# FDzhaozi/HiD-VAE

Measured on AMD Instinct MI355X. Metric: item-embeddings/sec HiD-VAE train step, 768-d in, 3x256 codebooks, higher is better.
Workload: dtype f32; 1 GPU; Amazon-Beauty-shaped synthetic 768-d, 3x256 codebooks, batch 1024/GPU, ROTATION_TRICK, tagged (projector+InfoNCE+predictor+focal/mixup: the step both h-configs run) train step = fwd+bwd+AdamW(cosine); global_batch=1024, parallelism=dp1, hip_graph=True, graph_queues=3, GPU_MAX_HW_QUEUES=4, collectives_in_graph=False

## Files before the change

hid-vae_amd/_C.py:

```python
import ctypes
import os

import torch

_HERE = os.path.dirname(os.path.abspath(__file__))
LIB_PATH = os.path.join(_HERE, "libhidvae_hip.so")
_lib = None

MODE_GUMBEL, MODE_STE, MODE_ROTATION = 1, 2, 3
DIST_L2, DIST_COSINE = 0, 1
GEMM_NT, GEMM_NN, GEMM_TN = 0, 1, 2
EPI_NONE, EPI_SILU, EPI_RELU, EPI_GELU, EPI_SIGMOID = 0, 1, 2, 3, 4
EPI_DSILU, EPI_DRELU, EPI_DGELU, EPI_DSIGMOID = 16, 17, 18, 19
MAX_LEVELS = 8
EMBED_DIM = 32

_vp, _i, _i64, _f, _u32 = ctypes.c_void_p, ctypes.c_int, ctypes.c_int64, ctypes.c_float, ctypes.c_uint32

_SIGNATURES = {
    "hidvae_gemm_f32": [_i, _i64, _i64, _i64, _vp, _i64, _vp, _i64, _vp, _vp, _i64, _i, _vp, _i64, _vp, _i64, _f, _vp, _u32, _u32, _i, _vp, _i, _vp],
    "hidvae_linear_bwd": [_vp, _i64, _vp, _i64, _vp, _i64, _i64, _i64, _i64, _vp, _i64, _i, _vp, _i64, _i, _vp, _i64, _f, _vp, _i, _vp, _i, _vp],
    "hidvae_layernorm_bwd_partial": [_vp, _vp, _vp, _vp, _vp, _vp, _i64, _i64, _i, _vp, _f, _f, _vp, _vp, _vp, _vp, _vp],
    "hidvae_layernorm_param_final_many": [_vp, _i, _vp],
    "hidvae_predictor_fwd": [_vp, _i64, _i64, _vp, _i, _vp, _vp],
    "hidvae_predictor_bwd": [_vp, _i64, _i64, _vp, _i, _vp, _i64, _vp],
    "hidvae_gate_fwd": [_vp, _i64, _i64, _i, _vp, _vp, _vp, _vp, _vp, _vp, _i, _f, _vp, _vp, _vp, _vp, _vp, _vp, _vp],
    "hidvae_gate_bwd": [_vp, _i64, _vp, _i64, _i64, _i, _vp, _vp, _vp, _i, _f, _vp, _vp, _vp, _vp, _vp, _vp, _vp, _vp, _vp],
    "hidvae_colsum": [_vp, _i64, _i64, _i64, _vp, _i, _vp, _vp],
    "hidvae_codebook_prepare": [_vp, _vp, _i, _i64, _vp, _vp, _i, _vp],
    "hidvae_rq_forward": [_vp, _i64, _i, _vp, _vp, _i, _i64, _i, _i, _f, _vp, _vp, _vp, _i64, _vp, _vp, _vp, _vp, _i, _i, _vp],
    "hidvae_bottleneck_fwd": [_vp, _i64, _i, _i, _vp, _vp, _vp, _vp, _vp, _i, _vp, _vp, _i, _i64, _i, _f, _vp, _vp, _vp, _i64, _vp, _vp,
                              _i, _i, _vp, _vp, _vp, _vp, _vp, _vp, _vp, _vp, _vp, _vp],
    "hidvae_rq_backward": [_vp, _vp, _i64, _i, _vp, _vp, _i, _i64, _i, _f, _vp, _vp, _i64, _vp, _vp, _i64, _f, _vp, _i64, _vp, _vp, _i, _vp],
    "hidvae_rq_backward_slices": [_vp, _vp, _i64, _i, _vp, _vp, _i, _i64, _i, _f, _vp, _vp, _vp, _i, _vp, _vp, _i64, _f, _vp, _i64, _vp, _vp, _i, _vp],
    "hidvae_uniq_loss": [_vp, _vp, _i64, _i, _f, _f, _vp, _vp, _i, _vp],
    "hidvae_total_loss": [_vp, _vp, _i64, _vp, _vp, _vp, _i, _f, _vp, _vp, _i, _f, _f, _f, _f, _f, _vp, _vp, _vp, _vp, _vp, _i, _vp],
    "hidvae_total_loss_bwd": [_vp, _i64, _i, _f, _f, _f, _vp, _vp, _vp, _i, _vp],
    "hidvae_codebook_grad": [_vp, _vp, _i64, _i, _i64, _vp, _vp, _vp, _vp, _i, _vp, _i, _vp],
    "hidvae_l2norm_fwd_pair": [_vp, _i64, _i64, _vp, _vp, _vp, _i64, _i64, _vp, _vp, _i64, _f, _vp],
    "hidvae_l2norm_bwd_pair": [_vp, _i64, _vp, _vp, _i64, _vp, _vp, _i64, _vp, _vp, _i64, _vp, _i64, _f, _vp],
    "hidvae_recon_fwd_bwd": [_vp, _vp, _i64, _i64, _i, _f, _vp, _i64, _vp, _vp, _vp, _vp],
    "hidvae_l2norm_fwd": [_vp, _i64, _i64, _i64, _f, _vp, _i64, _vp, _vp],
    "hidvae_l2norm32_fwd": [_vp, _i64, _i64, _f, _vp, _i64, _vp, _vp],
    "hidvae_l2norm_bwd": [_vp, _i64, _vp, _i64, _vp, _i64, _i64, _f, _vp, _i64, _i, _vp],
    "hidvae_id_stats": [_vp, _i64, _vp, _i64, _i, _vp, _vp, _vp, _i, _vp],
    "hidvae_act_bwd": [_vp, _vp, _i64, _i, _vp, _f, _vp, _vp],
    "hidvae_binary": [_i, _vp, _i64, _vp, _i64, _i64, _i64, _vp, _i64, _vp],
    "hidvae_sum_prefix_slices": [_vp, _vp, _i, _i64, _i64, _vp, _vp],
    "hidvae_layernorm_fwd": [_vp, _i64, _i64, _vp, _vp, _f, _vp, _vp, _vp, _i, _vp, _f, _vp, _vp, _u32, _u32, _vp],
    "hidvae_rng_advance": [_vp, _vp],
    "hidvae_dropout_mask": [_vp, _i64, _vp, _u32, _u32, _vp],
    "hidvae_layernorm_bwd": [_vp, _vp, _vp, _vp, _vp, _vp, _i64, _i64, _i, _vp, _f, _vp, _vp],
    "hidvae_layernorm_param_grad": [_vp, _vp, _vp, _vp, _vp, _vp, _i64, _i64, _i, _vp, _f, _vp, _vp, _i, _vp, _vp],
    "hidvae_layernorm_bwd_all": [_vp, _vp, _vp, _vp, _vp, _vp, _i64, _i64, _i, _vp, _f, _vp, _vp, _vp, _i, _vp, _vp],
    "hidvae_batchnorm_fwd": [_vp, _i64, _i64, _i64, _vp, _vp, _f, _f, _i, _vp, _vp, _vp, _vp, _vp, _vp, _i, _vp, _f, _vp, _u32, _u32, _vp, _vp],
    "hidvae_batchnorm_bwd": [_vp, _vp, _i64, _vp, _vp, _vp, _vp, _i64, _i64, _i, _vp, _f, _vp, _vp, _vp, _vp, _i, _vp, _vp],
    "hidvae_infonce_rows": [_vp, _i64, _f, _f, _vp, _vp, _vp],
    "hidvae_infonce_dlogits": [_vp, _i64, _f, _f, _vp, _vp],
    "hidvae_infonce_lse_chunk": [_vp, _i64, _i64, _i64, _i64, _f, _vp, _vp, _vp, _i, _vp],
    "hidvae_infonce_lse_finish": [_vp, _vp, _vp, _i64, _f, _f, _vp, _vp, _vp, _vp],
    "hidvae_infonce_dlogits_chunk": [_vp, _i64, _i64, _i64, _i64, _f, _f, _vp, _vp, _vp],
    "hidvae_mixup_plan": [_vp, _i64, _i, _i64, _vp, _f, _vp, _vp, _vp, _vp, _vp],
    "hidvae_tag_loss_fwd": [_vp, _i64, _i64, _vp, _vp, _vp, _i, _f, _f, _f, _f, _vp, _vp, _vp, _vp, _vp, _vp, _vp, _vp, _vp],
    "hidvae_tag_loss_bwd": [_vp, _vp, _vp, _vp, _vp, _i64, _i64, _vp, _vp, _vp, _vp],
    "hidvae_kmeans_iter": [_vp, _i64, _vp, _i64, _vp, _vp, _vp, _vp, _vp, _i, _vp],
    "hidvae_gumbel_rows_fwd": [_vp, _vp, _vp, _vp, _i64, _i64, _f, _vp, _i, _i, _vp],
    "hidvae_gumbel_loss": [_vp, _vp, _i64, _f, _vp, _i, _vp],
    "hidvae_gumbel_gemb": [_vp, _vp, _i64, _vp, _vp, _i64, _vp, _i, _vp],
    "hidvae_gumbel_rows_bwd": [_vp, _vp, _i64, _i64, _f, _vp, _vp],
    "hidvae_gumbel_finish": [_vp, _vp, _vp, _vp, _vp, _i64, _f, _i64, _vp, _vp, _vp, _i64, _i, _vp],
    "hidvae_cat_recon_rows": [_vp, _i64, _vp, _i64, _i64, _i64, _i, _vp, _i64, _vp, _vp, _vp],
    "hidvae_loss_fwd": [_vp, _vp, _i64, _i64, _i, _vp, _vp, _vp, _vp, _i, _f, _vp, _vp, _i, _f, _f, _f, _f, _f, _vp, _vp, _vp, _vp, _vp, _vp, _i, _vp],
    "hidvae_loss_bwd": [_vp, _vp, _vp, _i64, _i64, _i, _i, _f, _f, _f, _vp, _vp, _vp, _vp, _i, _f, _vp],
    "hidvae_padded_to_jagged": [_vp, _i64, _i64, _vp, _vp, _i64, _i64, _i64, _vp],
    "hidvae_jagged_to_padded": [_vp, _vp, _vp, _i64, _i64, _i64, _i64, _i64, _vp],
    "hidvae_gather_rows": [_vp, _i64, _i, _vp, _vp, _vp, _vp, _vp],
    "hidvae_codebook_prepare_adamw": [_vp, _vp, _i, _i64, _vp, _vp, _vp, _vp, _vp, _i, _f, _f, _f, _i64, _i64, _f, _vp, _i, _vp],
    "hidvae_adamw_prepare": [_vp, _vp, _vp, _i, _f, _f, _f, _i64, _i64, _f, _vp, _vp],
    "hidvae_adamw_step": [_vp, _vp, _vp, _vp, _vp, _vp, _i, _i64, _f, _f, _f, _f, _vp],
    "hidvae_query_workspace": [_i, _vp, _i, _vp],
    "hidvae_sqdiff_rows": [_vp, _i64, _vp, _i64, _i64, _i64, _f, _vp, _vp],
    "hidvae_sqdiff_rows_bwd": [_vp, _i64, _vp, _i64, _vp, _i64, _i64, _i64, _f, _f, _vp, _vp, _vp],
    "hidvae_gumbel_noise": [_vp, _i64, _f, _vp, _vp],
    "hidvae_gumbel_softmax_rows": [_vp, _vp, _i64, _i64, _f, _vp, _vp],
    "hidvae_softmax_argmax_rows": [_vp, _i64, _i64, _i64, _vp, _i64, _vp, _i64, _vp],
    "hidvae_timestamp": [_vp, _vp],
    "hidvae_linear_bwd_group": [_vp, _i, _vp],
    "hidvae_gemm_bf16": [_i64, _i64, _i64, _vp, _i64, _vp, _i64, _vp, _vp, _i64, _i, _vp, _i64, _vp, _i64, _f, _vp, _u32, _u32, _vp, _i, _vp],
    "hidvae_linear_bwd_bf16": [_vp, _i64, _vp, _i64, _vp, _i64, _i64, _i64, _i64, _vp, _i64, _i, _vp, _i64, _i, _vp, _i64, _f, _vp, _i, _vp, _vp],
    "hidvae_linear_bwd_group_bf16": [_vp, _i, _vp],
}
WS_GEMM, WS_LINEAR_BWD, WS_COLSUM, WS_CODEBOOK_GRAD, WS_LAYERNORM_PARAM_GRAD, WS_LAYERNORM_BWD_ALL = 1, 2, 3, 4, 5, 6
WS_BATCHNORM_FWD, WS_BATCHNORM_BWD, WS_ID_CENSUS, WS_KMEANS, WS_TAG_LOSS, WS_LINEAR_BWD_ZEROED, WS_RQ_FORWARD = 7, 8, 9, 10, 11, 12, 13
WS_LINEAR_BWD_BF16, WS_GEMM_BF16, WS_BF16_ZEROED = 14, 15, 16
PRECISIONS = ("fp32", "bf16")


class LaunchStamps:
    TICK_US = 0.01

    def __init__(self, device, capacity=4096):
        self.buf = torch.zeros((2 * capacity,), dtype=torch.int64, device=device)
        self.names, self.dims = [], []
        self.streams = []

    def _slot(self, name, dims=None, stream=None):
        if 2 * len(self.names) + 2 > self.buf.numel():
            raise RuntimeError("LaunchStamps: capacity exceeded")
        self.names.append(name)
        self.dims.append(dims)
        self.streams.append(int(getattr(stream, "value", stream) or 0))
        return self.buf.data_ptr() + 16 * (len(self.names) - 1)

    def rows(self):
        t = self.buf[: 2 * len(self.names)].cpu().reshape(-1, 2)
        d = ((t[:, 1] - t[:, 0]).double() * self.TICK_US).tolist()
        empty = [v for n, v in zip(self.names, d) if n == "(empty)"]
        base = sorted(empty)[len(empty) // 2] if empty else 0.0
        return [(n, v - base) for n, v in zip(self.names, d) if n != "(empty)"], base

    def spans(self):
        t = self.buf[: 2 * len(self.names)].cpu().reshape(-1, 2).double() * self.TICK_US
        t0 = float(t[:, 0].min()) if len(self.names) else 0.0
        return [(n, s, float(a) - t0, float(b) - t0) for n, s, (a, b) in zip(self.names, self.streams, t.tolist()) if n != "(empty)"]

    def rows_with_dims(self):
        rows, base = self.rows()
        dims = [dm for n, dm in zip(self.names, self.dims) if n != "(empty)"]
        return [(n, v, dm) for (n, v), dm in zip(rows, dims)], base


class PhaseMarks:

    def __init__(self, device, capacity=512):
        self.buf = torch.zeros((capacity,), dtype=torch.int64, device=device)
        self.labels = []

    def rows(self):
        t = self.buf[: len(self.labels)].cpu().double() * LaunchStamps.TICK_US
        t0 = float(t.min()) if len(self.labels) else 0.0
        return [(lab, st, float(v) - t0) for (lab, st), v in zip(self.labels, t.tolist())]


_PHASES = None


def phases_begin(device, capacity=512):
    global _PHASES
    _PHASES = PhaseMarks(device, capacity)
    return _PHASES


def phases_end():
    global _PHASES
    p, _PHASES = _PHASES, None
    return p


def phase_mark(label):
    p = _PHASES
    if p is None:
        return
    i = len(p.labels)
    if i >= p.buf.numel():
        raise RuntimeError("PhaseMarks: capacity exceeded")
    st = torch.cuda.current_stream().cuda_stream
    p.labels.append((label, int(st)))
    lib()._L.hidvae_timestamp(ctypes.c_void_p(p.buf.data_ptr() + 8 * i), ctypes.c_void_p(st))


_STAMPS = None
_NOT_LAUNCHES = ("hidvae_last_error", "hidvae_version", "hidvae_query_workspace", "hidvae_timestamp")


def stamps_begin(device, capacity=4096):
    global _STAMPS
    _STAMPS = LaunchStamps(device, capacity)
    return _STAMPS


def stamps_end():
    global _STAMPS
    st, _STAMPS = _STAMPS, None
    return st


def stamp_empty_bracket():
    st = _STAMPS
    if st is not None:
        p = st._slot("(empty)")
        lib()._L.hidvae_timestamp(ctypes.c_void_p(p), _stream())
        lib()._L.hidvae_timestamp(ctypes.c_void_p(p + 8), _stream())


def _gemm_dims(name, a):
    if name == "hidvae_gemm_f32":
        return (int(a[1]), int(a[2]), int(a[3]), 2.0 * a[1] * a[2] * a[3])
    if name == "hidvae_gemm_bf16":
        return (int(a[0]), int(a[1]), int(a[2]), 2.0 * a[0] * a[1] * a[2])
    if name in ("hidvae_linear_bwd", "hidvae_linear_bwd_bf16"):
        B, n_out, n_in = int(a[6]), int(a[7]), int(a[8])
        return (B, n_out, n_in, (4.0 if a[12] is not None else 2.0) * B * n_out * n_in)
    if name == "hidvae_bottleneck_fwd":
        B, K2, N2, L, K, Nd0, Nd1 = int(a[1]), int(a[2]), int(a[3]), int(a[12]), int(a[13]), int(a[22]), int(a[23])
        D = EMBED_DIM
        return (B, N2, K2, 2.0 * B * (K2 * N2 + N2 * D + L * K * D + D * Nd0 + Nd0 * Nd1))
    return None


class _LibProxy:

    def __init__(self, L):
        self._L = L

    def __getattr__(self, name):
        fn = getattr(self._L, name)
        if name in _NOT_LAUNCHES or not name.startswith("hidvae_"):
            return fn
        L = self._L

        def call(*a):
            st = _STAMPS
            if st is None:
                return fn(*a)
            p = st._slot(name, _gemm_dims(name, a), a[-1])
            L.hidvae_timestamp(ctypes.c_void_p(p), a[-1])
            rc = fn(*a)
            L.hidvae_timestamp(ctypes.c_void_p(p + 8), a[-1])
            return rc

        setattr(self, name, call)
        return call


def lib():
    global _lib
    if _lib is None:
        if not os.path.exists(LIB_PATH):
            raise RuntimeError(
                f"HIP extension missing: {LIB_PATH}. Build it with `python -c 'import __graft_entry__ as g; g.build()'` "
                "(hipcc --offload-arch=gfx950). There is no CPU fallback on the product path.")
        L = ctypes.CDLL(LIB_PATH)
        L.hidvae_last_error.restype = ctypes.c_char_p
        L.hidvae_version.restype = ctypes.c_char_p
        for name, sig in _SIGNATURES.items():
            fn = getattr(L, name)
            fn.argtypes = sig
            fn.restype = ctypes.c_int
        _lib = _LibProxy(L)
    return _lib


def exported_symbols():
    return ["hidvae_version", "hidvae_last_error"] + list(_SIGNATURES)

# ... 1056 lines not shown
```

hid-vae_amd/csrc/gemm.hip:

```cpp
#include <stdlib.h>
#include <type_traits>
#include "common.h"
#include "rules.h"
#include "gemm_ring.h"

namespace {

constexpr int BK = 16;

struct GemmArgs {
    int64_t M, N, K;
    const float *A;
    int64_t lda;
    const float *B;
    int64_t ldb;
    const float *bias;
    float *C;
    int64_t ldc;
    int epilogue;
    float *aux;
    int64_t ldaux;
    int accumulate;
    int64_t k_per_split;
    float *partial;
// ... 1262 lines not shown
        for (int v = 0; v < NV; v++) {
            f32x4 x = pf[slot][v];
            const int k = s * T16_BKS + k4[v];
            if (k + 4 > Ki) {
#pragma unroll
                for (int e = 0; e < 4; e++) x[e] = k + e < Ki ? x[e] : 0.0f;
            }
            *reinterpret_cast<f32x4 *>(base + dst[v]) = x;
        }
    };
    f32x4 acc = {0.f, 0.f, 0.f, 0.f};
    f32x4 fa[2][4], fb[2][4];
    auto frags = [&](int fs, int buf) {
        const float *As = lds + buf * BUF + (16 * wm + i16) * T16_STR + 4 * q;
        const float *Bs = lds + buf * BUF + A_SZ + (16 * wn + i16) * T16_STR + 4 * q;
#pragma unroll
        for (int u = 0; u < 4; u++) {
            fa[fs][u] = *reinterpret_cast<const f32x4 *>(As + 16 * u);
            fb[fs][u] = *reinterpret_cast<const f32x4 *>(Bs + 16 * u);
        }
    };
#pragma unroll
    for (int p = 0; p < PF; p++) fetch(p, p);
    stash(0, 0, 0);
    fetch(0, PF);
    stash(1 % PF, 1, 1);
    fetch(1 % PF, PF + 1);
    __syncthreads();
    frags(0, 0);
    constexpr int UN = 6;
    for (int s0 = 0; s0 < nsteps; s0 += UN) {
#pragma unroll
        for (int u = 0; u < UN; u++) {
            const int s = s0 + u;
            if (s < nsteps) {
                const int nblk = (Ki - s * T16_BKS + 15) / 16;
#pragma unroll
                for (int s4 = 0; s4 < 4; s4++) acc = __builtin_amdgcn_mfma_f32_16x16x4f32(fa[u & 1][0][s4], fb[u & 1][0][s4], acc, 0, 0, 0);
                __builtin_amdgcn_sched_barrier(0);
                if (s + 1 < nsteps) frags((u + 1) & 1, (u + 1) % NB);
                __builtin_amdgcn_sched_barrier(0);
#pragma unroll
                for (int b = 1; b < 4; b++)
                    if (b < nblk) {
#pragma unroll
                        for (int s4 = 0; s4 < 4; s4++) acc = __builtin_amdgcn_mfma_f32_16x16x4f32(fa[u & 1][b][s4], fb[u & 1][b][s4], acc, 0, 0, 0);
                    }
                if (s + 2 < nsteps) {
                    stash((u + 2) % PF, s + 2, (u + 2) % NB);
                    fetch((u + 2) % PF, s + 2 + PF);
                }
                __syncthreads();
            }
        }
    }
    const int64_t col = n0 + 16 * wn + i16;
    if (col >= g.N) return;
    const float bias = g.bias != nullptr ? g.bias[col] : 0.0f;
    const float *mk = g.mask;
#pragma unroll
    for (int r = 0; r < 4; r++) {
        const int64_t row = m0 + 16 * wm + 4 * q + r;
        if (row >= g.M) continue;
        float v = acc[r] + bias;
        if (g.aux != nullptr && g.epilogue < HIDVAE_EPI_DSILU && g.epilogue != HIDVAE_EPI_NONE) g.aux[row * g.ldaux + col] = v;
        v = apply_epilogue(g.epilogue, v, g.aux, row * g.ldaux + col, g.mask_scale);
        if (has_dropout(g)) v = v * dropout_factor(g, row, col);
        float *dstp = g.C + row * g.ldc + col;
        *dstp = g.accumulate ? *dstp + v : v;
    }
}

template <int WM, int WN>
int launch_tile16(const GemmArgs &g, hipStream_t s) {
    constexpr size_t bytes = (size_t)3 * (16 * WM + 16 * WN) * T16_STR * 4;
    static const hipError_t attr = hipFuncSetAttribute(reinterpret_cast<const void *>(&gemm_tile16_kernel<WM, WN>),
                                                       hipFuncAttributeMaxDynamicSharedMemorySize, (int)bytes);
    if (attr != hipSuccess) return -1;
    const int64_t tiles = hv_cdiv(g.M, 16 * WM) * hv_cdiv(g.N, 16 * WN);
    hipLaunchKernelGGL((gemm_tile16_kernel<WM, WN>), dim3((unsigned)tiles), dim3(64 * WM * WN), bytes, s, g);
    return 0;
}

template <int SPLIT>
void launch_directL(int layout, const GemmArgs &g, hipStream_t s) {
    dim3 grid((unsigned)hv_cdiv(g.N, 32), (unsigned)hv_cdiv(g.M, 32));
    dim3 block(64 * SPLIT);
    if (layout == HIDVAE_GEMM_NT) hipLaunchKernelGGL((gemm_directL_kernel<HIDVAE_GEMM_NT, SPLIT>), grid, block, 0, s, g);
    else hipLaunchKernelGGL((gemm_directL_kernel<HIDVAE_GEMM_NN, SPLIT>), grid, block, 0, s, g);
}

template <int SPLIT, int NS, int NWN = 1>
void launch_direct(int layout, const GemmArgs &g, hipStream_t s) {
    dim3 grid((unsigned)hv_cdiv(hv_cdiv(g.N, 32), NWN), (unsigned)hv_cdiv(g.M, 32));
    dim3 block(64 * SPLIT * NWN);
    if (layout == HIDVAE_GEMM_NT) hipLaunchKernelGGL((gemm_direct_kernel<HIDVAE_GEMM_NT, SPLIT, NS, NWN>), grid, block, 0, s, g);
    else if (layout == HIDVAE_GEMM_NN) hipLaunchKernelGGL((gemm_direct_kernel<HIDVAE_GEMM_NN, SPLIT, NS, NWN>), grid, block, 0, s, g);
    else hipLaunchKernelGGL((gemm_direct_kernel<HIDVAE_GEMM_TN, SPLIT, NS, NWN>), grid, block, 0, s, g);
}

template <int WM, int WN>
void launch_tile(int layout, const GemmArgs &g, int splits, hipStream_t s) {
    dim3 grid((unsigned)hv_cdiv(g.N, 32 * WN), (unsigned)hv_cdiv(g.M, 32 * WM), (unsigned)splits);
    dim3 block(64 * WM * WN);
    if (layout == HIDVAE_GEMM_NT) hipLaunchKernelGGL((gemm_f32_kernel<WM, WN, HIDVAE_GEMM_NT>), grid, block, 0, s, g);
    else if (layout == HIDVAE_GEMM_NN) hipLaunchKernelGGL((gemm_f32_kernel<WM, WN, HIDVAE_GEMM_NN>), grid, block, 0, s, g);
    else hipLaunchKernelGGL((gemm_f32_kernel<WM, WN, HIDVAE_GEMM_TN>), grid, block, 0, s, g);
}

inline bool aligned16(const void *p) { return (reinterpret_cast<uintptr_t>(p) & 15) == 0; }

inline bool fits32bit(int layout, int64_t M, int64_t N, int64_t K, int64_t lda, int64_t ldb) {
    const int64_t a_rows = (layout == HIDVAE_GEMM_TN) ? K : M, b_rows = (layout == HIDVAE_GEMM_NT) ? N : K;
    return a_rows * lda < (1ll << 29) && b_rows * ldb < (1ll << 29);
}
inline bool use_direct16(int64_t M, int64_t N, int64_t K) {
    const int64_t tiles32 = hv_cdiv(M, 32) * hv_cdiv(N, 32);
    return tiles32 <= 256 || (tiles32 <= 512 && K <= 256);
}
inline int pick_split32(int64_t M, int64_t N, int64_t K, int split_k) {
    const int64_t tiles32 = hv_cdiv(M, 32) * hv_cdiv(N, 32);
    int sp = 1;
    if (split_k != 1) {
        const int cap = split_k == 0 ? 16 : split_k;
        while (sp < cap && sp < 16 && tiles32 * sp < 2048 && K / (sp * 2) >= 32) sp *= 2;
    }
    return sp;
}
inline int pick_split16(int64_t M, int64_t N, int64_t K, int split_k) {
    const int64_t tiles16 = hv_cdiv(M, 16) * hv_cdiv(N, 16);
    int sp16 = 1;
    if (split_k != 1) {
        const int cap = split_k == 0 ? 16 : split_k;
        while (sp16 < cap && sp16 < 16 && tiles16 * sp16 < 4096 && K / (sp16 * 2) >= 32) sp16 *= 2;
    }
    return sp16;
}

constexpr int GROUP_MAX = 12;
constexpr int GROUP_WAVES = 8;
struct GroupSub {
    GemmArgs g;
    int kind;
    int layout, split, deep, nbx;
    int64_t nt;
    int nb;
};
struct GroupArgs {
    int n;
    GroupSub s[GROUP_MAX];
};

__device__ __forceinline__ void colsum_group_body(const GemmArgs &g, int64_t c0, float *part) {
    const int col = threadIdx.x & 31, rg = threadIdx.x >> 5, nrg = (int)(blockDim.x >> 5);
    const int64_t c = c0 + col;
    float acc = 0.0f;
    if (c < g.N)
        for (int64_t r0 = rg; r0 < g.M; r0 += 8 * (int64_t)nrg) {
            float v[8];
#pragma unroll
            for (int j = 0; j < 8; j++) v[j] = r0 + (int64_t)nrg * j < g.M ? g.A[(r0 + (int64_t)nrg * j) * g.lda + c] : 0.0f;
#pragma unroll
            for (int j = 0; j < 8; j++) acc += v[j];
        }
    part[rg * 32 + col] = acc;
    __syncthreads();
    if (threadIdx.x < 32 && c < g.N) {
        float v = part[col];
        for (int j = 1; j < nrg; j++) v += part[j * 32 + col];
        g.C[c] = g.accumulate ? g.C[c] + v : v;
    }
}

__global__ __launch_bounds__(64 * GROUP_WAVES) void gemm_group_kernel(GroupArgs a) {
    __shared__ float part[GROUP_WAVES * 1024];
    int bid = blockIdx.x, p = 0;
    while (p + 1 < a.n && bid >= a.s[p].nb) {
        bid -= a.s[p].nb;
        p++;
    }
    const GroupSub &s = a.s[p];
    if (s.kind == 2) {
        colsum_group_body(s.g, (int64_t)bid * 32, part);
        return;
    }
    const int64_t tile0 = (int64_t)xcd_slot(bid, s.nb) * (GROUP_WAVES / s.split);
    if (s.kind == 0) {
        if (s.layout == HIDVAE_GEMM_NT) {
            if (s.deep) direct16_body<HIDVAE_GEMM_NT, 6>(s.g, s.split, tile0, s.nt, s.nbx, part);
            else direct16_body<HIDVAE_GEMM_NT, 3>(s.g, s.split, tile0, s.nt, s.nbx, part);
        } else if (s.layout == HIDVAE_GEMM_NN) direct16_body<HIDVAE_GEMM_NN, 3>(s.g, s.split, tile0, s.nt, s.nbx, part);
        else direct16_body<HIDVAE_GEMM_TN, 3>(s.g, s.split, tile0, s.nt, s.nbx, part);
    } else {
        if (s.layout == HIDVAE_GEMM_NT) {
            if (s.deep) direct32_body<HIDVAE_GEMM_NT, 6>(s.g, s.split, tile0, s.nt, s.nbx, part);
            else direct32_body<HIDVAE_GEMM_NT, 3>(s.g, s.split, tile0, s.nt, s.nbx, part);
        } else if (s.layout == HIDVAE_GEMM_NN) {
            if (s.deep) direct32_body<HIDVAE_GEMM_NN, 6>(s.g, s.split, tile0, s.nt, s.nbx, part);
            else direct32_body<HIDVAE_GEMM_NN, 3>(s.g, s.split, tile0, s.nt, s.nbx, part);
        } else direct32_body<HIDVAE_GEMM_TN, 3>(s.g, s.split, tile0, s.nt, s.nbx, part);
    }
}

inline bool group_gemm_sub(GroupSub &s, int layout, const GemmArgs &g) {
    if (!fits32bit(layout, g.M, g.N, g.K, g.lda, g.ldb) || hv_cdiv(g.M, 32) * hv_cdiv(g.N, 32) >= 2048) return false;
    s.g = g;
    s.layout = layout;
    const bool f16 = use_direct16(g.M, g.N, g.K);
    s.kind = f16 ? 0 : 1;
    int sp = f16 ? pick_split16(g.M, g.N, g.K, 0) : pick_split32(g.M, g.N, g.K, 0);
    const int cap = hv_cdiv(g.M, 16) * hv_cdiv(g.N, 16) <= 16 ? GROUP_WAVES : 4;
    if (sp > GROUP_WAVES) sp = GROUP_WAVES;
    while (sp > cap && sp > 1) sp /= 2;
    s.split = sp;
    s.deep = g.K / (16 * sp) >= 12;
    const int T = f16 ? 16 : 32;
    s.nbx = (int)hv_cdiv(g.N, T);
    s.nt = (int64_t)s.nbx * hv_cdiv(g.M, T);
    s.nb = (int)hv_cdiv(s.nt, GROUP_WAVES / sp);
    return true;
}

inline int launch_group(GroupArgs &a, hipStream_t s) {
    int64_t blocks = 0;
    for (int i = 0; i < a.n; i++) blocks += a.s[i].nb;
    if (blocks == 0) return HIDVAE_OK;
    hipLaunchKernelGGL(gemm_group_kernel, dim3((unsigned)blocks), dim3(64 * GROUP_WAVES), 0, s, a);
    HV_LAUNCH_CHECK("gemm_group");
    return HIDVAE_OK;
}

}

extern "C" int hidvae_gemm_f32(int layout, int64_t M, int64_t N, int64_t K, const float *A, int64_t lda,
                               const float *B, int64_t ldb, const float *bias, float *C, int64_t ldc, int epilogue,
                               float *aux, int64_t ldaux, const float *mask, int64_t ldmask, float mask_scale,
                               const unsigned long long *rng_state, unsigned rng_site, unsigned drop_threshold,
                               int split_k, float *workspace, int accumulate, void *stream) {
    HV_REQUIRE(layout >= 0 && layout <= 2, "gemm: layout %d", layout);
    HV_REQUIRE(!(mask && rng_state), "gemm: a keep-mask OR the in-kernel generator, not both");
    HV_REQUIRE(M >= 1 && N >= 1 && K >= 1, "gemm: empty problem M=%lld N=%lld K=%lld", (long long)M, (long long)N, (long long)K);
    HV_REQUIRE(A && B && C, "gemm: null operand");
    const int64_t a_min = (layout == HIDVAE_GEMM_TN) ? M : K, b_min = (layout == HIDVAE_GEMM_NT) ? K : N;
    HV_REQUIRE(lda >= a_min && ldb >= b_min && ldc >= N, "gemm: leading dimension too small (lda=%lld ldb=%lld ldc=%lld)",
               (long long)lda, (long long)ldb, (long long)ldc);
    HV_REQUIRE(epilogue < HIDVAE_EPI_DSILU || (aux != nullptr && ldaux >= N), "gemm: backward epilogue %d needs aux", epilogue);
    HV_REQUIRE(mask == nullptr || ldmask >= N, "gemm: ldmask=%lld", (long long)ldmask);
    HV_REQUIRE(split_k >= 0, "gemm: split_k=%d", split_k);
    GemmArgs g{};
    g.M = M; g.N = N; g.K = K; g.A = A; g.lda = lda; g.B = B; g.ldb = ldb; g.bias = bias; g.C = C; g.ldc = ldc;
    g.epilogue = epilogue; g.aux = aux; g.ldaux = aux ? ldaux : 0; g.accumulate = accumulate;
    g.vecA = (lda % 4 == 0) && aligned16(A);
    g.vecB = (ldb % 4 == 0) && aligned16(B);
    g.mask = mask; g.ldmask = ldmask; g.mask_scale = mask_scale;
    g.drop = HvDrop{rng_state, rng_site, drop_threshold};
    hipStream_t s = (hipStream_t)stream;
    const int64_t tiles32 = hv_cdiv(M, 32) * hv_cdiv(N, 32);
    const bool fits32 = fits32bit(layout, M, N, K, lda, ldb);
    int deep_splits = 0;
    if (split_k == 0 && workspace != nullptr && K >= 4096 && tiles32 < 2048 && M > 32 && N > 32) {
        deep_splits = (int)(K / 512 < 16 ? K / 512 : 16);
        const int64_t wgs = hv_cdiv(M, 64) * hv_cdiv(N, 64);
        while (deep_splits > 2 && wgs * deep_splits > 2048) deep_splits /= 2;
    }
    const bool big = (tiles32 >= 2048 && K >= 64) || !fits32 || deep_splits > 1;
    if (!big || split_k == 1) {
        if (!big) {
            const int64_t nt16 = hv_cdiv(M, 16) * hv_cdiv(N, 16);
            const int64_t t_small = hv_cdiv(M, 32) * hv_cdiv(N, 64), t_big = hv_cdiv(M, 64) * hv_cdiv(N, 64);
            const bool fit_small = t_small >= 192 && t_small <= 256, fit_big = t_big >= 224 && t_big <= 256;
            if (layout == HIDVAE_GEMM_NT && split_k == 0 && K >= 256 && tiles32 >= 448) {
                HV_REQUIRE((launch_tile16<4, 4>(g, s)) == 0, "gemm_f32: could not size the LDS of gemm_tile16_kernel");
                HV_LAUNCH_CHECK("gemm_f32 tile16");
                return HIDVAE_OK;
            }
            if (layout == HIDVAE_GEMM_NT && split_k == 1 && K >= 256 && (fit_small || fit_big)) {
                const int rc = !fit_small ? launch_tile16<4, 4>(g, s) : launch_tile16<2, 4>(g, s);
                HV_REQUIRE(rc == 0, "gemm_f32: could not size the LDS of gemm_tile16_kernel");
                HV_LAUNCH_CHECK("gemm_f32 tile16");
                return HIDVAE_OK;
            }
            if (layout == HIDVAE_GEMM_NT && nt16 >= 512 && nt16 <= 8192 && K >= 64 && (split_k == 1 || (use_direct16(M, N, K) && K >= 128))) {
                constexpr int W16 = 4;
                hipLaunchKernelGGL(gemm_directL16_kernel<W16>, dim3((unsigned)hv_cdiv(nt16, W16)), dim3(64 * W16), 0, s, g);
                HV_LAUNCH_CHECK("gemm_f32 directL16");
                return HIDVAE_OK;
            }
            if (use_direct16(M, N, K)) {
                const int sp16 = pick_split16(M, N, K, split_k);
                const bool deep16 = K / (16 * sp16) >= 12;
                switch (sp16) {
                    case 1: if (deep16) launch_direct16<1, 6>(layout, g, s); else launch_direct16<1, 3>(layout, g, s); break;
                    case 2: if (deep16) launch_direct16<2, 6>(layout, g, s); else launch_direct16<2, 3>(layout, g, s); break;
                    case 4: if (deep16) launch_direct16<4, 6>(layout, g, s); else launch_direct16<4, 3>(layout, g, s); break;
                    case 8: launch_direct16<8, 3>(layout, g, s); break;
                    default: launch_direct16<16, 3>(layout, g, s); break;
                }
                HV_LAUNCH_CHECK("gemm_f32 direct16");
                return HIDVAE_OK;
            }
            const int sp = pick_split32(M, N, K, split_k);
            if (layout != HIDVAE_GEMM_TN && sp <= 8 && (sp >= 2 || tiles32 >= 1024)) {
                switch (sp) {
                    case 1: launch_directL<1>(layout, g, s); break;
                    case 2: launch_directL<2>(layout, g, s); break;
                    case 4: launch_directL<4>(layout, g, s); break;
                    default: launch_directL<8>(layout, g, s); break;
                }
                HV_LAUNCH_CHECK("gemm_f32 directL");
                return HIDVAE_OK;
            }
            const bool deep = K / (16 * sp) >= 12;
            switch (sp) {
                case 1: if (deep) launch_direct<1, 6>(layout, g, s); else launch_direct<1, 3>(layout, g, s); break;
                case 2: if (deep) launch_direct<2, 6>(layout, g, s); else launch_direct<2, 3>(layout, g, s); break;
                case 4: if (deep) launch_direct<4, 6>(layout, g, s); else launch_direct<4, 3>(layout, g, s); break;
                case 8: launch_direct<8, 3>(layout, g, s); break;
                default: launch_direct<16, 3>(layout, g, s); break;
            }
            HV_LAUNCH_CHECK("gemm_f32 direct");
            return HIDVAE_OK;
        }
    }
    int splits = (split_k > 1 && workspace != nullptr) ? split_k : (deep_splits > 1 ? deep_splits : 1);
    int64_t kps = hv_cdiv(hv_cdiv(K, splits), BK) * BK;
    splits = (int)hv_cdiv(K, kps);
    g.k_per_split = kps;
    g.partial = splits > 1 ? workspace : nullptr;
    if (N <= 32) launch_tile<2, 1>(layout, g, splits, s);
    else if (M <= 32) launch_tile<1, 2>(layout, g, splits, s);
    else launch_tile<2, 2>(layout, g, splits, s);
    HV_LAUNCH_CHECK("gemm_f32 tiled");
    if (splits > 1) {
        hipLaunchKernelGGL(splitk_reduce_kernel, dim3((unsigned)hv_cdiv(M * N, 256)), dim3(256), 0, s, g, splits);
        HV_LAUNCH_CHECK("splitk_reduce");
    }
    return HIDVAE_OK;
}

extern "C" int hidvae_colsum(const float *X, int64_t M, int64_t N, int64_t ldx, float *out, int accumulate, float *workspace, void *stream);

static int linear_bwd_impl(const float *g, int64_t ldg, const float *x, int64_t ldx, const float *W, int64_t ldw, int64_t B,
                           int64_t n_out, int64_t n_in, float *dW, int64_t lddw, int accumulate_dw, float *dX, int64_t lddx,
                           int dx_epilogue, float *aux, int64_t ldaux, float dx_scale, float *db, int accumulate_db, float *workspace,
                           void *stream, bool balanced_ok, bool co_resident = false) {
    HV_REQUIRE(g && x && dW && B >= 1 && n_out >= 1 && n_in >= 1, "linear_bwd: bad arguments");
    HV_REQUIRE(ldg >= n_out && ldx >= n_in && lddw >= n_in, "linear_bwd: leading dimension too small");
    HV_REQUIRE(dX == nullptr || (W != nullptr && ldw >= n_in && lddx >= n_in), "linear_bwd: dX needs W");
    HV_REQUIRE(dX == nullptr || dx_epilogue == HIDVAE_EPI_NONE || (dx_epilogue >= HIDVAE_EPI_DSILU && aux != nullptr && ldaux >= n_in),
               "linear_bwd: dX epilogue %d", dx_epilogue);
    const bool small = dX != nullptr && fits32bit(HIDVAE_GEMM_TN, n_out, n_in, B, ldg, ldx) && fits32bit(HIDVAE_GEMM_NN, B, n_in, n_out, ldg, ldw) &&
                       hv_cdiv(n_out, 32) * hv_cdiv(n_in, 32) < 2048 && hv_cdiv(B, 32) * hv_cdiv(n_in, 32) < 2048;
    const bool pair16 = small && use_direct16(n_out, n_in, B) && use_direct16(B, n_in, n_out);
    const int s32_0 = pick_split32(n_out, n_in, B, 0), s32_1 = pick_split32(B, n_in, n_out, 0);
    const bool pair32 = small && !use_direct16(n_out, n_in, B) && !use_direct16(B, n_in, n_out) && s32_0 <= 8 && s32_1 <= 8;
    const bool pair = pair16 || pair32;
    constexpr int mid_minq = 6;
    if (balanced_ok && workspace != nullptr && hv_lbwd_balanced(B, n_out, n_in, true) &&
        fits32bit(HIDVAE_GEMM_TN, n_out, n_in, B, ldg, ldx) && (dX == nullptr || fits32bit(HIDVAE_GEMM_NN, B, n_in, n_out, ldg, ldw))) {
        if (dX == nullptr || ldg == n_out || n_out % 4 == 0) {
            const int rc = hv_ring_linear_bwd(g, ldg, x, ldx, W, ldw, B, n_out, n_in, dW, lddw, accumulate_dw, dX, lddx, dx_epilogue, aux, ldaux,
                                              dx_scale, db, accumulate_db, workspace, 512, (hipStream_t)stream);
            if (rc != 1) return rc;
        }
        auto run_mid = [&](auto kg_tag) -> int {
        constexpr int KG = decltype(kg_tag)::value, BKS = 16 * KG;
        SkArgs a{};
        PairArgs &p = a.p;
        p.g0.M = n_out; p.g0.N = n_in; p.g0.K = B; p.g0.A = g; p.g0.lda = ldg; p.g0.B = x; p.g0.ldb = ldx; p.g0.C = dW; p.g0.ldc = lddw;
        p.g0.epilogue = HIDVAE_EPI_NONE; p.g0.mask_scale = 1.0f; p.g0.accumulate = accumulate_dw;
        p.nbx0 = (int)hv_cdiv(n_in, 64);
        p.nb0 = p.nbx0 * (int)hv_cdiv(n_out, 64);
        a.n0 = (int)hv_cdiv(B, BKS);
        if (dX != nullptr) {
            p.g1.M = B; p.g1.N = n_in; p.g1.K = n_out; p.g1.A = g; p.g1.lda = ldg; p.g1.B = W; p.g1.ldb = ldw; p.g1.C = dX; p.g1.ldc = lddx;
            p.g1.epilogue = dx_epilogue; p.g1.aux = aux; p.g1.ldaux = aux ? ldaux : 0; p.g1.mask_scale = dx_scale;
            p.nbx1 = (int)hv_cdiv(n_in, 64);
            p.nb1 = p.nbx1 * (int)hv_cdiv(B, 64);
            a.n1 = (int)hv_cdiv(n_out, BKS);
        } else a.n1 = 1;
        p.cs_x = g; p.cs_ld = ldg; p.cs_rows = B; p.cs_cols = n_out; p.cs_out = db; p.cs_accumulate = accumulate_db;
        a.nbc = db != nullptr ? (int)hv_cdiv(n_out, 32) : 0;
        a.cu = (int)hv_cdiv(B, 128 * KG);
        a.S = p.nb0 * a.n0 + p.nb1 * a.n1 + a.nbc * a.cu;
        constexpr int slots = 1024 / KG;
        int G = a.S / mid_minq;
        if (G > slots) G = slots;
        if (G < 1) G = 1;
        a.q = (int)hv_cdiv(a.S, G);
        a.G = (int)hv_cdiv(a.S, a.q);
        const int longest = a.n0 > (p.nb1 ? a.n1 : 0) ? a.n0 : a.n1;
        const bool tiles = p.nb0 + p.nb1 + a.nbc <= slots && longest * KG <= 96;
        if (tiles) {
            a.q = 0;
            a.G = p.nb0 + p.nb1 + a.nbc;
        }
        if (p.nb0 + p.nb1 <= HV_SK_COUNTERS && (tiles || a.G <= HV_SK_MAX_G)) {
            a.counters = reinterpret_cast<int *>(workspace);
            a.slabs = workspace + HV_SK_COUNTERS;
            const int rc = launch_mid_sk<KG, 2>(a, (hipStream_t)stream);
            HV_REQUIRE(rc == 0, "linear_bwd: could not size the LDS of gemm_mid_sk_kernel");
            HV_LAUNCH_CHECK("linear_bwd mid");
            return HIDVAE_OK;
        }
        return 1;
        };
        int rc_mid = co_resident ? run_mid(std::integral_constant<int, 2>{}) : 1;
        if (rc_mid == 1) rc_mid = run_mid(std::integral_constant<int, 4>{});
        if (rc_mid != 1) return rc_mid;
    }
    if (balanced_ok && workspace != nullptr && hv_lbwd_balanced(B, n_out, n_in, true)) workspace += HV_SK_COUNTERS;
    HV_REQUIRE(db == nullptr || pair || workspace != nullptr || B <= 16384, "linear_bwd: the unpaired bias gradient needs the colsum workspace");
    if (!pair) {
        int rc = HIDVAE_OK;
        if (db != nullptr) rc = hidvae_colsum(g, B, n_out, ldg, db, accumulate_db, workspace, stream);
        if (rc == HIDVAE_OK)
            rc = hidvae_gemm_f32(HIDVAE_GEMM_TN, n_out, n_in, B, g, ldg, x, ldx, nullptr, dW, lddw, HIDVAE_EPI_NONE, nullptr, 0, nullptr, 0,
                                 1.0f, nullptr, 0u, 0u, 0, workspace, accumulate_dw, stream);
        if (rc != HIDVAE_OK || dX == nullptr) return rc;
        return hidvae_gemm_f32(HIDVAE_GEMM_NN, B, n_in, n_out, g, ldg, W, ldw, nullptr, dX, lddx, dx_epilogue, aux, ldaux, nullptr, 0, dx_scale,
                               nullptr, 0u, 0u, 0, nullptr, 0, stream);
    }
// ... 100 lines not shown
```

hid-vae_amd/csrc/rules.h:

```cpp
#pragma once
#include <stdint.h>

constexpr int64_t HV_SK_COUNTERS = 4096;
constexpr int64_t HV_SK_MAX_G = 512;
constexpr int64_t HV_SK_WS_FLOATS = HV_SK_COUNTERS + HV_SK_MAX_G * 2 * 4096;

static inline bool hv_lbwd_balanced(int64_t B, int64_t n_out, int64_t n_in, bool has_dx = true) {
    const int64_t t64 = ((n_out + 63) / 64) * ((n_in + 63) / 64), u64 = ((B + 63) / 64) * ((n_in + 63) / 64);
    const double mflop = 2.0e-6 * (double)B * (double)n_out * (double)n_in * (has_dx ? 2.0 : 1.0);
    constexpr double min_mflop = 200.0;
    constexpr int64_t max_b = 16384;
    return n_out >= 64 && n_in >= 64 && B >= 256 && B <= max_b && t64 + u64 <= HV_SK_COUNTERS && mflop >= min_mflop;
}
```

include/hidvae.h:

```cpp
#ifndef HIDVAE_H
#define HIDVAE_H
#include <stdint.h>

#ifdef __cplusplus
extern "C" {
#endif

#define HIDVAE_OK 0
#define HIDVAE_EINVAL (-1)
#define HIDVAE_EUNSUPPORTED (-2)
#define HIDVAE_ELAUNCH (-3)

#define HIDVAE_MAX_LEVELS 8

#define HIDVAE_MODE_GUMBEL 1
#define HIDVAE_MODE_STE 2
#define HIDVAE_MODE_ROTATION 3

#define HIDVAE_DIST_L2 0
#define HIDVAE_DIST_COSINE 1

#define HIDVAE_GEMM_NT 0
#define HIDVAE_GEMM_NN 1
#define HIDVAE_GEMM_TN 2

#define HIDVAE_EPI_NONE 0
#define HIDVAE_EPI_SILU 1
#define HIDVAE_EPI_RELU 2
#define HIDVAE_EPI_GELU 3
#define HIDVAE_EPI_SIGMOID 4
#define HIDVAE_EPI_DSILU 16
#define HIDVAE_EPI_DRELU 17
#define HIDVAE_EPI_DGELU 18
#define HIDVAE_EPI_DSIGMOID 19

const char *hidvae_version(void);
const char *hidvae_last_error(void);

#define HIDVAE_WS_GEMM 1
#define HIDVAE_WS_LINEAR_BWD 2
#define HIDVAE_WS_COLSUM 3
#define HIDVAE_WS_CODEBOOK_GRAD 4
#define HIDVAE_WS_LAYERNORM_PARAM_GRAD 5
#define HIDVAE_WS_LAYERNORM_BWD_ALL 6
#define HIDVAE_WS_BATCHNORM_FWD 7
#define HIDVAE_WS_BATCHNORM_BWD 8
#define HIDVAE_WS_ID_CENSUS 9
#define HIDVAE_WS_KMEANS 10
#define HIDVAE_WS_TAG_LOSS 11
#define HIDVAE_WS_RQ_FORWARD 13
#define HIDVAE_WS_LINEAR_BWD_ZEROED 12
#define HIDVAE_WS_LINEAR_BWD_BF16 14
#define HIDVAE_WS_GEMM_BF16 15
#define HIDVAE_WS_BF16_ZEROED 16
int hidvae_query_workspace(int op, const int64_t *dims, int n_dims, int64_t *bytes);

int hidvae_gemm_f32(int layout, int64_t M, int64_t N, int64_t K,
                    const float *A, int64_t lda, const float *B, int64_t ldb,
                    const float *bias, float *C, int64_t ldc,
                    int epilogue, float *aux, int64_t ldaux,
                    const float *mask, int64_t ldmask, float mask_scale,
                    const unsigned long long *rng_state, unsigned rng_site, unsigned drop_threshold,
                    int split_k, float *workspace, int accumulate, void *stream);

int hidvae_linear_bwd(const float *g, int64_t ldg, const float *x, int64_t ldx, const float *W, int64_t ldw, int64_t B,
                      int64_t n_out, int64_t n_in, float *dW, int64_t lddw, int accumulate_dw, float *dX, int64_t lddx,
                      int dx_epilogue, float *aux, int64_t ldaux, float dx_scale, float *db, int accumulate_db, float *workspace,
                      int co_resident, void *stream);

typedef struct {
    const float *g; int64_t ldg;
    const float *x; int64_t ldx;
    const float *W; int64_t ldw;
    int64_t B, n_out, n_in;
    float *dW; int64_t lddw; int accumulate_dw;
    float *dX; int64_t lddx;
    int dx_epilogue;
    float *aux; int64_t ldaux;
    float *db; int accumulate_db;
    float *workspace;
} hidvae_linear_bwd_problem;
int hidvae_linear_bwd_group(const hidvae_linear_bwd_problem *problems_host, int n, void *stream);

int hidvae_gemm_bf16(int64_t M, int64_t N, int64_t K,
                     const float *A, int64_t lda, const float *B, int64_t ldb,
                     const float *bias, float *C, int64_t ldc,
                     int epilogue, float *aux, int64_t ldaux,
                     const float *mask, int64_t ldmask, float mask_scale,
                     const unsigned long long *rng_state, unsigned rng_site, unsigned drop_threshold,
                     float *workspace, int accumulate, void *stream);

int hidvae_linear_bwd_bf16(const float *g, int64_t ldg, const float *x, int64_t ldx, const float *W, int64_t ldw, int64_t B,
                           int64_t n_out, int64_t n_in, float *dW, int64_t lddw, int accumulate_dw, float *dX, int64_t lddx,
                           int dx_epilogue, float *aux, int64_t ldaux, float dx_scale, float *db, int accumulate_db, float *workspace,
                           void *stream);

int hidvae_linear_bwd_group_bf16(const hidvae_linear_bwd_problem *problems_host, int n, void *stream);

int hidvae_colsum(const float *X, int64_t M, int64_t N, int64_t ldx, float *out, int accumulate,
                  float *workspace, void *stream);

int hidvae_codebook_prepare(const float *const *E_host, const int32_t *normalize_host, int L, int64_t K,
                            float *cb_eff, float *cc, int embed_dim, void *stream);

int hidvae_rq_forward(const float *y, int64_t B, int normalize_input,
                      const float *cb_eff, const float *cc, int L, int64_t K,
                      int mode, int training, float beta,
                      float *z, int64_t *ids, float *emb_cat, int64_t ld_cat,
                      float *emb_sum, float *res_cat, float *qloss, void *workspace, int embed_dim, int distance, void *stream);

int hidvae_bottleneck_fwd(const float *h1, int64_t B, int K2, int N2, const float *W2, const float *W3, float *pre2, float *h2,
                          float *y, int normalize_input, const float *cb_eff, const float *cc, int L, int64_t K, int mode,
                          float beta, float *z, int64_t *ids, float *emb_cat, int64_t ld_cat, float *emb_sum, float *qloss,
                          int Nd0, int Nd1, const float *Wd0, const float *Wd1, float *pre_d0, float *d0, float *pre_d1,
                          float *d1, float *embs_norm, float *p_unique, int64_t *census_scratch, void *stream);

int hidvae_rq_backward(const float *y, const float *z, int64_t B, int normalize_input,
                       const float *cb_eff, const float *cc, int L, int64_t K,
                       int mode, float beta, const int64_t *ids,
                       const float *g_cat, int64_t ld_gcat, const float *g_sum, const float *g_z_in,
                       int64_t g_z_rows, float gq, const float *gq_items, int64_t gq_stride, float *g_y, float *dE_rows, int embed_dim, void *stream);
int hidvae_rq_backward_slices(const float *y, const float *z, int64_t B, int normalize_input, const float *cb_eff, const float *cc,
                              int L, int64_t K, int mode, float beta, const int64_t *ids, const float *const *g_slices_host,
                              const int32_t *slice_width_host, int n_slices, const float *g_sum, const float *g_z_in,
                              int64_t g_z_rows, float gq, const float *gq_items, int64_t gq_stride, float *g_y, float *dE_rows,
                              int embed_dim, void *stream);

int hidvae_codebook_grad(const int64_t *ids, const float *dE_rows, int64_t B, int L, int64_t K,
                         const float *const *E_host, const float *cb_eff, const int32_t *normalize_host,
                         float *const *gE_host, int accumulate, float *workspace, int embed_dim, void *stream);

int hidvae_recon_fwd_bwd(const float *y, const float *x, int64_t B, int64_t N, int n_cat, float gscale,
                         const float *gscale_items, int64_t gs_stride, float *x_hat, float *recon, float *g_y,
                         void *stream);

int hidvae_l2norm_fwd(const float *x, int64_t M, int64_t N, int64_t ldx, float eps, float *out, int64_t ldo,
                      float *norms, void *stream);
int hidvae_l2norm32_fwd(const float *x, int64_t M, int64_t ldx, float eps, float *out, int64_t ldo, float *norms,
                        void *stream);
int hidvae_l2norm_bwd(const float *g, int64_t ldg, const float *out, int64_t ldo, const float *norms,
                      int64_t M, int64_t N, float eps, float *gx, int64_t ldgx, int accumulate, void *stream);
int hidvae_l2norm_fwd_pair(const float *x0, int64_t ldx0, int64_t N0, float *out0, float *norms0, const float *x1, int64_t ldx1, int64_t N1,
                           float *out1, float *norms1, int64_t M, float eps, void *stream);
int hidvae_l2norm_bwd_pair(const float *g0, int64_t ldg0, const float *out0, const float *norms0, int64_t N0, float *gx0, const float *g1,
                           int64_t ldg1, const float *out1, const float *norms1, int64_t N1, float *gx1, int64_t M, float eps, void *stream);

// ... 154 lines not shown
```

Measured before the change: 1.001 million items/s.

## Add whole-tile pipelined MFMA GEMM for large forward NT problems

```diff
diff --git a/hid-vae_amd/_C.py b/hid-vae_amd/_C.py
--- a/hid-vae_amd/_C.py
+++ b/hid-vae_amd/_C.py
@@ -19,6 +19,7 @@
 
 _SIGNATURES = {
     "hidvae_gemm_f32": [_i, _i64, _i64, _i64, _vp, _i64, _vp, _i64, _vp, _vp, _i64, _i, _vp, _i64, _vp, _i64, _f, _vp, _u32, _u32, _i, _vp, _i, _vp],
+    "hidvae_gemm_f32_wholetile": [_i64, _i64, _i64, _i],
     "hidvae_linear_bwd": [_vp, _i64, _vp, _i64, _vp, _i64, _i64, _i64, _i64, _vp, _i64, _i, _vp, _i64, _i, _vp, _i64, _f, _vp, _i, _vp, _i, _vp],
     "hidvae_layernorm_bwd_partial": [_vp, _vp, _vp, _vp, _vp, _vp, _i64, _i64, _i, _vp, _f, _f, _vp, _vp, _vp, _vp, _vp],
     "hidvae_layernorm_param_final_many": [_vp, _i, _vp],
@@ -170,7 +171,7 @@
 
 
 _STAMPS = None
-_NOT_LAUNCHES = ("hidvae_last_error", "hidvae_version", "hidvae_query_workspace", "hidvae_timestamp")
+_NOT_LAUNCHES = ("hidvae_last_error", "hidvae_version", "hidvae_query_workspace", "hidvae_timestamp", "hidvae_gemm_f32_wholetile")
 
 
 def stamps_begin(device, capacity=4096):
diff --git a/hid-vae_amd/csrc/gemm.hip b/hid-vae_amd/csrc/gemm.hip
--- a/hid-vae_amd/csrc/gemm.hip
+++ b/hid-vae_amd/csrc/gemm.hip
@@ -1368,6 +1368,195 @@
     return 0;
 }
 
+constexpr int WT_BK = 32;
+#define WT_LDSP(p) ((__attribute__((address_space(3))) void *)(p))
+
+template <int TM, int TN, int WM, int WN, int D>
+struct WtGeom {
+    static constexpr int NS = D + 1;
+    static constexpr int RM = TM / (16 * WM), RN = TN / (16 * WN);
+    static constexpr int NP = (TM + TN) / 8;
+    static constexpr int NI = (NP + 3) / 4;
+    static constexpr int STAGE = NI * 4 * 256;
+    static constexpr size_t LDS_BYTES = (size_t)NS * STAGE * 4;
+    static_assert(WM * WN == 4 && TM % (16 * WM) == 0 && TN % (16 * WN) == 0, "four waves, whole 16x16 sub-tiles");
+    static_assert(TM % 32 == 0 && TN % 8 == 0, "a round of four pieces lies in one operand's image");
+};
+
+template <int R, int NI>
+__device__ __forceinline__ void wt_wait_tail(int rem) {
+    if constexpr (R > 0) {
+        if (rem == R) asm volatile("s_waitcnt vmcnt(%0)" : : "n"(R * NI) : "memory");
+        else wt_wait_tail<R - 1, NI>(rem);
+    } else asm volatile("s_waitcnt vmcnt(0)" : : : "memory");
+}
+
+template <int TM, int TN, int WM, int WN, int D>
+__global__ __launch_bounds__(256) void gemm_wt_kernel(GemmArgs g) {
+    using G = WtGeom<TM, TN, WM, WN, D>;
+    constexpr int RM = G::RM, RN = G::RN, NI = G::NI;
+    extern __shared__ __attribute__((aligned(16))) float wt_lds[];
+    float *lds = wt_lds;
+    const int lane = threadIdx.x & 63;
+    const int wave = __builtin_amdgcn_readfirstlane(threadIdx.x >> 6);
+    const int wm = wave / WN, wn = wave - wm * WN;
+    const int i16 = lane & 15, q = lane >> 4;
+    const int nbx = (int)((g.N + TN - 1) / TN), nby = (int)((g.M + TM - 1) / TM);
+    const int tile = xcd_slot((int)blockIdx.x, nbx * nby);
+    const int bx = tile / nby, by = tile - bx * nby;
+    const int m0 = by * TM, n0 = bx * TN;
+    const int Mi = (int)g.M, Ni = (int)g.N, Ki = (int)g.K;
+    const int nsteps = (Ki + WT_BK - 1) / WT_BK;
+    const __amdgpu_buffer_rsrc_t ra = __builtin_amdgcn_make_buffer_rsrc(const_cast<float *>(g.A), 0, (int)(4 * ((g.M - 1) * g.lda + g.K)), 0x00020000);
+    const __amdgpu_buffer_rsrc_t rb = __builtin_amdgcn_make_buffer_rsrc(const_cast<float *>(g.B), 0, (int)(4 * ((g.N - 1) * g.ldb + g.K)), 0x00020000);
+    int voff[NI], kc[NI];
+#pragma unroll
+    for (int i = 0; i < NI; i++) {
+        const bool isA = i < TM / 32;
+        const int p = wave + 4 * i;
+        const int r = 8 * p + (lane >> 3) - (isA ? 0 : TM);
+        const int c = (lane & 7) ^ ((r >> 1) & 7);
+        const int row = (isA ? m0 : n0) + r;
+        kc[i] = 4 * c;
+        voff[i] = (p < G::NP && row < (isA ? Mi : Ni)) ? 4 * (row * (int)(isA ? g.lda : g.ldb) + 4 * c) : HV_OOB;
+    }
+    auto issue = [&](int s, int buf) {
+        float *dst = lds + buf * G::STAGE;
+#pragma unroll
+        for (int i = 0; i < NI; i++) {
+            const int v = (voff[i] != HV_OOB && s * WT_BK + kc[i] < Ki) ? voff[i] + s * (4 * WT_BK) : HV_OOB;
+            __builtin_amdgcn_raw_ptr_buffer_load_lds(i < TM / 32 ? ra : rb, WT_LDSP(dst + 256 * (wave + 4 * i)), 16, v, 0, 0, 0);
+        }
+    };
+    f32x4 acc[RM][RN];
+#pragma unroll
+    for (int i = 0; i < RM; i++)
+#pragma unroll
+        for (int j = 0; j < RN; j++) acc[i][j] = f32x4{0.f, 0.f, 0.f, 0.f};
+    const int sw = (i16 >> 1) & 7;
+    const int offA = (16 * RM * wm + i16) * WT_BK, offB = TM * WT_BK + (16 * RN * wn + i16) * WT_BK;
+    struct Frags {
+        f32x4 a[2][RM], b[2][RN];
+    };
+    auto fetch = [&](int s, Frags &f, auto edge) {
+        const float *st = lds + (s % G::NS) * G::STAGE;
+        const int kv = Ki - s * WT_BK;
+#pragma unroll
+        for (int b = 0; b < 2; b++) {
+            const int ch = 4 * ((4 * b + q) ^ sw);
+#pragma unroll
+            for (int i = 0; i < RM; i++) f.a[b][i] = *reinterpret_cast<const f32x4 *>(st + offA + 16 * WT_BK * i + ch);
+#pragma unroll
+            for (int j = 0; j < RN; j++) f.b[b][j] = *reinterpret_cast<const f32x4 *>(st + offB + 16 * WT_BK * j + ch);
+        }
+        if (decltype(edge)::value && kv < WT_BK) {
+#pragma unroll
+            for (int b = 0; b < 2; b++)
+#pragma unroll
+                for (int e = 0; e < 4; e++)
+                    if (16 * b + 4 * q + e >= kv) {
+#pragma unroll
+                        for (int i = 0; i < RM; i++) f.a[b][i][e] = 0.0f;
+#pragma unroll
+                        for (int j = 0; j < RN; j++) f.b[b][j][e] = 0.0f;
+                    }
+        }
+    };
+    auto mma = [&](int s, const Frags &f, auto edge) {
+        const int kv = Ki - s * WT_BK;
+#pragma unroll
+        for (int b = 0; b < 2; b++) {
+            if (decltype(edge)::value && 16 * b >= kv) break;
+#pragma unroll
+            for (int s4 = 0; s4 < 4; s4++)
+#pragma unroll
+                for (int i = 0; i < RM; i++)
+#pragma unroll
+                    for (int j = 0; j < RN; j++) acc[i][j] = __builtin_amdgcn_mfma_f32_16x16x4f32(f.a[b][i][s4], f.b[b][j][s4], acc[i][j], 0, 0, 0);
+        }
+    };
+    auto landed = [&](int younger) {
+        if (younger >= D - 1) asm volatile("s_waitcnt vmcnt(%0)" : : "n"((D - 1) * NI) : "memory");
+        else wt_wait_tail<D - 2, NI>(younger);
+    };
+    auto iter = [&](int s, const Frags &cur, Frags &nxt, auto edge) {
+        const int last = s + D - 1 < nsteps - 1 ? s + D - 1 : nsteps - 1;
+        landed(last - (s + 1));
+        __builtin_amdgcn_s_barrier();
+        if (s + D < nsteps) issue(s + D, (s + D) % G::NS);
+        fetch(s + 1, nxt, edge);
+        __builtin_amdgcn_sched_barrier(0);
+        mma(s, cur, std::false_type{});
+    };
+#pragma unroll
+    for (int i = 0; i < D; i++)
+        if (i < nsteps) issue(i, i);
+    Frags f0, f1;
+    landed((nsteps < D ? nsteps : D) - 1);
+    __builtin_amdgcn_s_barrier();
+    if (nsteps == 1) fetch(0, f0, std::true_type{});
+    else fetch(0, f0, std::false_type{});
+    int s = 0;
+    for (; s + 5 < nsteps; s += 4) {
+        iter(s, f0, f1, std::false_type{});
+        iter(s + 1, f1, f0, std::false_type{});
+        iter(s + 2, f0, f1, std::false_type{});
+        iter(s + 3, f1, f0, std::false_type{});
+    }
+    if (s + 3 < nsteps) {
+        iter(s, f0, f1, std::false_type{});
+        iter(s + 1, f1, f0, std::false_type{});
+        s += 2;
+    }
+    const int left = nsteps - s;
+    if (left == 1) {
+        mma(s, f0, std::true_type{});
+    } else if (left == 2) {
+        iter(s, f0, f1, std::true_type{});
+        mma(s + 1, f1, std::true_type{});
+    } else {
+        iter(s, f0, f1, std::false_type{});
+        iter(s + 1, f1, f0, std::true_type{});
+        mma(s + 2, f0, std::true_type{});
+    }
+#pragma unroll
+    for (int j = 0; j < RN; j++) {
+        const int64_t col = n0 + 16 * (RN * wn + j) + i16;
+        if (col >= g.N) continue;
+        const float bias = g.bias != nullptr ? g.bias[col] : 0.0f;
+#pragma unroll
+        for (int i = 0; i < RM; i++)
+#pragma unroll
+            for (int r = 0; r < 4; r++) {
+                const int64_t row = m0 + 16 * (RM * wm + i) + 4 * q + r;
+                if (row >= g.M) continue;
+                float v = acc[i][j][r] + bias;
+                if (g.aux != nullptr && g.epilogue < HIDVAE_EPI_DSILU && g.epilogue != HIDVAE_EPI_NONE) g.aux[row * g.ldaux + col] = v;
+                v = apply_epilogue(g.epilogue, v, g.aux, row * g.ldaux + col, g.mask_scale);
+                if (has_dropout(g)) v = v * dropout_factor(g, row, col);
+                float *dstp = g.C + row * g.ldc + col;
+                *dstp = g.accumulate ? *dstp + v : v;
+            }
+    }
+}
+
+constexpr int WT_D = 3;
+
+template <int TM, int TN, int WM, int WN>
+int launch_wt(const GemmArgs &g, hipStream_t s) {
+    using G = WtGeom<TM, TN, WM, WN, WT_D>;
+    static const hipError_t attr = hipFuncSetAttribute(reinterpret_cast<const void *>(&gemm_wt_kernel<TM, TN, WM, WN, WT_D>),
+                                                       hipFuncAttributeMaxDynamicSharedMemorySize, (int)G::LDS_BYTES);
+    if (attr != hipSuccess) return -1;
+    const int64_t tiles = hv_cdiv(g.M, TM) * hv_cdiv(g.N, TN);
+    hipLaunchKernelGGL((gemm_wt_kernel<TM, TN, WM, WN, WT_D>), dim3((unsigned)tiles), dim3(256), G::LDS_BYTES, s, g);
+    return 0;
+}
+
+inline int launch_wt_form(int form, const GemmArgs &g, hipStream_t s) {
+    return form == HV_WT_64x32 ? launch_wt<64, 32, 2, 2>(g, s) : launch_wt<32, 64, 2, 2>(g, s);
+}
+
 template <int SPLIT>
 void launch_directL(int layout, const GemmArgs &g, hipStream_t s) {
     dim3 grid((unsigned)hv_cdiv(g.N, 32), (unsigned)hv_cdiv(g.M, 32));
@@ -1421,6 +1610,15 @@
         while (sp16 < cap && sp16 < 16 && tiles16 * sp16 < 4096 && K / (sp16 * 2) >= 32) sp16 *= 2;
     }
     return sp16;
+}
+
+inline int wholetile_route(int64_t M, int64_t N, int64_t K, int split_k) {
+    static const bool on = [] {
+        const char *e = getenv("HIDVAE_FWD_WHOLETILE");
+        return !(e != nullptr && e[0] == '0' && e[1] == '\0');
+    }();
+    if (!on || split_k != 0 || K < 256 || hv_cdiv(M, 32) * hv_cdiv(N, 32) < 448) return -1;
+    return hv_fwd_wholetile(M, N, K);
 }
 
 constexpr int GROUP_MAX = 12;
@@ -1555,6 +1753,14 @@
             const int64_t nt16 = hv_cdiv(M, 16) * hv_cdiv(N, 16);
             const int64_t t_small = hv_cdiv(M, 32) * hv_cdiv(N, 64), t_big = hv_cdiv(M, 64) * hv_cdiv(N, 64);
             const bool fit_small = t_small >= 192 && t_small <= 256, fit_big = t_big >= 224 && t_big <= 256;
+            if (layout == HIDVAE_GEMM_NT) {
+                const int form = wholetile_route(M, N, K, split_k);
+                if (form >= 0) {
+                    HV_REQUIRE(launch_wt_form(form, g, s) == 0, "gemm_f32: could not size the LDS of gemm_wt_kernel");
+                    HV_LAUNCH_CHECK("gemm_f32 wholetile");
+                    return HIDVAE_OK;
+                }
+            }
             if (layout == HIDVAE_GEMM_NT && split_k == 0 && K >= 256 && tiles32 >= 448) {
                 HV_REQUIRE((launch_tile16<4, 4>(g, s)) == 0, "gemm_f32: could not size the LDS of gemm_tile16_kernel");
                 HV_LAUNCH_CHECK("gemm_f32 tile16");
@@ -1624,6 +1830,12 @@
     return HIDVAE_OK;
 }
 
+extern "C" int hidvae_gemm_f32_wholetile(int64_t M, int64_t N, int64_t K, int split_k) {
+    const bool direct = M >= 1 && N >= 1 && K >= 1 && K < 4096 && !(hv_cdiv(M, 32) * hv_cdiv(N, 32) >= 2048 && K >= 64) &&
+                        fits32bit(HIDVAE_GEMM_NT, M, N, K, K, K);
+    return direct ? wholetile_route(M, N, K, split_k) : -1;
+}
+
 extern "C" int hidvae_colsum(const float *X, int64_t M, int64_t N, int64_t ldx, float *out, int accumulate, float *workspace, void *stream);
 
 static int linear_bwd_impl(const float *g, int64_t ldg, const float *x, int64_t ldx, const float *W, int64_t ldw, int64_t B,
diff --git a/hid-vae_amd/csrc/rules.h b/hid-vae_amd/csrc/rules.h
--- a/hid-vae_amd/csrc/rules.h
+++ b/hid-vae_amd/csrc/rules.h
@@ -12,3 +12,22 @@
     constexpr int64_t max_b = 16384;
     return n_out >= 64 && n_in >= 64 && B >= 256 && B <= max_b && t64 + u64 <= HV_SK_COUNTERS && mflop >= min_mflop;
 }
+
+enum { HV_WT_64x32 = 0, HV_WT_32x64 = 1, HV_WT_FORMS = 2 };
+constexpr int64_t HV_WT_SLOTS = 256;
+
+static inline int hv_fwd_wholetile(int64_t M, int64_t N, int64_t K) {
+    static const int tm[HV_WT_FORMS + 1] = {64, 32, 64}, tn[HV_WT_FORMS + 1] = {32, 64, 64};
+    if (K < 256) return -1;
+    int best = HV_WT_FORMS;
+    int64_t best_cost = 0, best_bytes = 0, best_wgs = 0;
+    for (int f = HV_WT_FORMS; f >= 0; f--) {
+        const int64_t wgs = ((M + tm[f] - 1) / tm[f]) * ((N + tn[f] - 1) / tn[f]);
+        const int64_t cost = ((wgs + HV_WT_SLOTS - 1) / HV_WT_SLOTS) * tm[f] * tn[f], bytes = wgs * (tm[f] + tn[f]);
+        if (f == HV_WT_FORMS || cost < best_cost || (cost == best_cost && bytes < best_bytes)) {
+            best = f; best_cost = cost; best_bytes = bytes; best_wgs = wgs;
+        }
+    }
+    const int64_t rounds = (best_wgs + HV_WT_SLOTS - 1) / HV_WT_SLOTS;
+    return best < HV_WT_FORMS && 4 * best_wgs >= 3 * rounds * HV_WT_SLOTS ? best : -1;
+}
diff --git a/include/hidvae.h b/include/hidvae.h
--- a/include/hidvae.h
+++ b/include/hidvae.h
@@ -62,6 +62,8 @@
                     const float *mask, int64_t ldmask, float mask_scale,
                     const unsigned long long *rng_state, unsigned rng_site, unsigned drop_threshold,
                     int split_k, float *workspace, int accumulate, void *stream);
+
+int hidvae_gemm_f32_wholetile(int64_t M, int64_t N, int64_t K, int split_k);
 
 int hidvae_linear_bwd(const float *g, int64_t ldg, const float *x, int64_t ldx, const float *W, int64_t ldw, int64_t B,
                       int64_t n_out, int64_t n_in, float *dW, int64_t lddw, int accumulate_dw, float *dX, int64_t lddx,
```

New measurement: 989,900 items/s, median of 2. 0.989x the previous value.
